# microsoft/NOTSOFAR1-Challenge

Hardware: AMD Instinct MI355X
Metric: CSS real-time-factor (sep. audio sec/wall sec) on 7-ch 16 kHz (higher is better)
Workload: dtype f32 (float32 operands on v_mfma_f32_32x32x2_f32 in every Linear layer, attention product and transform: the reference's own operand precision; MVDR covariance / solve f64)

## Files before the change

notsofar1-challenge_amd/csrc/encoder.hip:

```cpp
#include "kernels.hpp"
#include "split_f16.hpp"

namespace css {

typedef float f32x16 __attribute__((ext_vector_type(16)));
typedef _Float16 f16x8 __attribute__((ext_vector_type(8)));

template <int CTRL>
__device__ __forceinline__ float dpp_addf(float v) {
    return v + __int_as_float(__builtin_amdgcn_update_dpp(0, __float_as_int(v), CTRL, 0xf, 0xf, false));
}
__device__ __forceinline__ float wave_sum(float v) {
    v = dpp_addf<0xB1>(v);
    v = dpp_addf<0x4E>(v);
    v = dpp_addf<0x141>(v);
    v = dpp_addf<0x140>(v);
    const float r0 = __int_as_float(__builtin_amdgcn_readlane(__float_as_int(v), 0));
    const float r1 = __int_as_float(__builtin_amdgcn_readlane(__float_as_int(v), 16));
    const float r2 = __int_as_float(__builtin_amdgcn_readlane(__float_as_int(v), 32));
    const float r3 = __int_as_float(__builtin_amdgcn_readlane(__float_as_int(v), 48));
    return (r0 + r1) + (r2 + r3);
}

#ifndef CSS_LN_ROWS
#define CSS_LN_ROWS 4
#endif
constexpr int LN_ROWS = CSS_LN_ROWS;
template <int NV, int MODE>
__global__ __launch_bounds__(64 * LN_ROWS) void layernorm_kernel(const float* __restrict__ x, float* __restrict__ y,
                                                        float* __restrict__ ys, const float* __restrict__ w,
                                                        const float* __restrict__ b, const float* __restrict__ pw,
                                                        int rows) {
    constexpr int D = 256 * NV;
    const int row = blockIdx.x * LN_ROWS + (threadIdx.x >> 6);
    if (row >= rows) return;
    const int lane = threadIdx.x & 63;
    const float4* xr = reinterpret_cast<const float4*>(x + (int64_t)row * D);
    float4 v[NV];
    float s = 0.f;
#pragma unroll
    for (int i = 0; i < NV; ++i) {
        v[i] = xr[lane + 64 * i];
        s += (v[i].x + v[i].y) + (v[i].z + v[i].w);
    }
    const float mean = wave_sum(s) * (1.0f / D);
    float q = 0.f;
#pragma unroll
    for (int i = 0; i < NV; ++i) {
        v[i].x -= mean; v[i].y -= mean; v[i].z -= mean; v[i].w -= mean;
        q += (v[i].x * v[i].x + v[i].y * v[i].y) + (v[i].z * v[i].z + v[i].w * v[i].w);
    }
    const float rstd = 1.0f / sqrtf(wave_sum(q) * (1.0f / D) + 1e-5f);
    float p0 = 0.f, p1 = 0.f, p2 = 0.f, p3 = 0.f;
    if (MODE == 2) { p0 = pw[0]; p1 = pw[1]; p2 = pw[2]; p3 = pw[3]; }
    float4* yr = reinterpret_cast<float4*>(y + (int64_t)row * D);
    _Float16* ysr = reinterpret_cast<_Float16*>(ys + (int64_t)row * D);
#pragma unroll
    for (int i = 0; i < NV; ++i) {
        const float4 g = reinterpret_cast<const float4*>(w)[lane + 64 * i];
        const float4 be = reinterpret_cast<const float4*>(b)[lane + 64 * i];
        float o[4] = {v[i].x * rstd * g.x + be.x, v[i].y * rstd * g.y + be.y, v[i].z * rstd * g.z + be.z,
                      v[i].w * rstd * g.w + be.w};
#pragma unroll
        for (int e = 0; e < 4; ++e) {
            if (MODE == 1) o[e] = fmaxf(o[e], 0.f);
            if (MODE == 2) o[e] = (p0 * o[e] + p1) * (1.0f / (1.0f + expf(-(p2 * o[e] + p3))));
        }
        if (y) yr[lane + 64 * i] = make_float4(o[0], o[1], o[2], o[3]);
        if (ys) split_store4(ysr, 4 * (lane + 64 * i), o[0], o[1], o[2], o[3]);
    }
}

template <int NV>
__global__ __launch_bounds__(64 * LN_ROWS) void layernorm2_kernel(const float* __restrict__ x, float* __restrict__ y,
                                                         const float* __restrict__ w1, const float* __restrict__ b1,
                                                         float* __restrict__ z, float* __restrict__ zs,
                                                         const float* __restrict__ w2, const float* __restrict__ b2,
                                                         int rows) {
    constexpr int D = 256 * NV;
    const int row = blockIdx.x * LN_ROWS + (threadIdx.x >> 6);
    if (row >= rows) return;
    const int lane = threadIdx.x & 63;
    const float4* xr = reinterpret_cast<const float4*>(x + (int64_t)row * D);
    float4 v[NV];
#pragma unroll
    for (int i = 0; i < NV; ++i) v[i] = xr[lane + 64 * i];
#pragma unroll
    for (int pass = 0; pass < 2; ++pass) {
        float s = 0.f;
#pragma unroll
        for (int i = 0; i < NV; ++i) s += (v[i].x + v[i].y) + (v[i].z + v[i].w);
        const float mean = wave_sum(s) * (1.0f / D);
        float q = 0.f;
#pragma unroll
        for (int i = 0; i < NV; ++i) {
            v[i].x -= mean; v[i].y -= mean; v[i].z -= mean; v[i].w -= mean;
            q += (v[i].x * v[i].x + v[i].y * v[i].y) + (v[i].z * v[i].z + v[i].w * v[i].w);
        }
        const float rstd = 1.0f / sqrtf(wave_sum(q) * (1.0f / D) + 1e-5f);
        const float* w = pass ? w2 : w1;
        const float* b = pass ? b2 : b1;
        float* yo = pass ? z : y;
#pragma unroll
        for (int i = 0; i < NV; ++i) {
            const float4 g = reinterpret_cast<const float4*>(w)[lane + 64 * i];
            const float4 be = reinterpret_cast<const float4*>(b)[lane + 64 * i];
            v[i] = make_float4(v[i].x * rstd * g.x + be.x, v[i].y * rstd * g.y + be.y, v[i].z * rstd * g.z + be.z,
                               v[i].w * rstd * g.w + be.w);
            if (yo) reinterpret_cast<float4*>(yo + (int64_t)row * D)[lane + 64 * i] = v[i];
            if (pass && zs)
                split_store4(reinterpret_cast<_Float16*>(zs + (int64_t)row * D), 4 * (lane + 64 * i), v[i].x, v[i].y, v[i].z, v[i].w);
        }
    }
}

void launch_layernorm2(const float* x, float* y, const float* w1, const float* b1, float* z, float* z_split,
                       const float* w2, const float* b2, int rows, int D, hipStream_t s) {
    const dim3 grid((rows + LN_ROWS - 1) / LN_ROWS), block(64 * LN_ROWS);
    switch (D) {
        case 256: hipLaunchKernelGGL((layernorm2_kernel<1>), grid, block, 0, s, x, y, w1, b1, z, z_split, w2, b2, rows); break;
        case 512: hipLaunchKernelGGL((layernorm2_kernel<2>), grid, block, 0, s, x, y, w1, b1, z, z_split, w2, b2, rows); break;
        case 768: hipLaunchKernelGGL((layernorm2_kernel<3>), grid, block, 0, s, x, y, w1, b1, z, z_split, w2, b2, rows); break;
        case 1024: hipLaunchKernelGGL((layernorm2_kernel<4>), grid, block, 0, s, x, y, w1, b1, z, z_split, w2, b2, rows); break;
        default: break;
    }
}

template <int MODE>
static void launch_ln_mode(const float* x, float* y, float* ys, const float* w, const float* b, const float* pw,
                           int rows, int D, hipStream_t s) {
    const dim3 grid((rows + LN_ROWS - 1) / LN_ROWS), block(64 * LN_ROWS);
    switch (D) {
        case 256: hipLaunchKernelGGL((layernorm_kernel<1, MODE>), grid, block, 0, s, x, y, ys, w, b, pw, rows); break;
        case 512: hipLaunchKernelGGL((layernorm_kernel<2, MODE>), grid, block, 0, s, x, y, ys, w, b, pw, rows); break;
        case 768: hipLaunchKernelGGL((layernorm_kernel<3, MODE>), grid, block, 0, s, x, y, ys, w, b, pw, rows); break;
        case 1024: hipLaunchKernelGGL((layernorm_kernel<4, MODE>), grid, block, 0, s, x, y, ys, w, b, pw, rows); break;
        default: break;
    }
}

void launch_layernorm(const float* x, float* y, float* y_split, const float* w, const float* b, int rows, int D,
                      int relu, hipStream_t s) {
    if (relu) launch_ln_mode<1>(x, y, y_split, w, b, nullptr, rows, D, s);
    else launch_ln_mode<0>(x, y, y_split, w, b, nullptr, rows, D, s);
}

void launch_ln_glu(const float* x, float* z, const float* w, const float* b, const float* pw, int rows, int D,
                   hipStream_t s) {
    launch_ln_mode<2>(x, z, nullptr, w, b, pw, rows, D, s);
}

template <int TAPS, int RUN>
__global__ __launch_bounds__(256) void dwconv_kernel(const float* __restrict__ z, float* __restrict__ h,
                                                     const float* __restrict__ wt, const float* __restrict__ dwb,
                                                     const float* __restrict__ alpha, const float* __restrict__ beta,
                                                     const float* __restrict__ pw, int T, int D, int runs_per_seg) {
    constexpr int PAD = (TAPS - 1) / 2;
    const int ch = blockIdx.x * 256 + threadIdx.x;
    if (ch >= D) return;
    const int seg = blockIdx.y / runs_per_seg, run = blockIdx.y % runs_per_seg;
    const int t0 = run * RUN;
    const float* zs = z + (int64_t)seg * T * D + ch;
    float wk[TAPS];
#pragma clang loop unroll(full)
    for (int k = 0; k < TAPS; ++k) wk[k] = wt[k * D + ch];
    float acc[RUN];
#pragma clang loop unroll(full)
    for (int j = 0; j < RUN; ++j) acc[j] = 0.f;
#pragma clang loop unroll(full)
    for (int p = 0; p < RUN + TAPS - 1; ++p) {
        const int t = t0 + p - PAD;
        const float v = (t >= 0 && t < T) ? zs[(int64_t)t * D] : 0.f;
#pragma clang loop unroll(full)
        for (int j = (p - (TAPS - 1) > 0 ? p - (TAPS - 1) : 0); j <= (p < RUN - 1 ? p : RUN - 1); ++j)
            acc[j] = fmaf(wk[p - j], v, acc[j]);
    }
    const float bb = dwb[ch], al = alpha[ch], be = beta[ch], w2 = pw[4], c2 = pw[5];
    float* hs = h + (int64_t)seg * T * D + ch;
#pragma unroll
    for (int j = 0; j < RUN; ++j) {
        const int t = t0 + j;
        if (t < T) {
            const float y = fmaxf((acc[j] + bb) * al + be, 0.f);
            hs[(int64_t)t * D] += w2 * y + c2;
        }
    }
}

void launch_dwconv(const float* z, float* h, const float* dw_wt, const float* dw_b, const float* bn_alpha,
                   const float* bn_beta, const float* pw, int nseg, int T, int D, int taps, hipStream_t s) {
    constexpr int RUN = 31;
    const int runs = (T + RUN - 1) / RUN;
    const dim3 grid((D + 255) / 256, nseg * runs), block(256);
    if (taps == 33)
        hipLaunchKernelGGL((dwconv_kernel<33, RUN>), grid, block, 0, s, z, h, dw_wt, dw_b, bn_alpha, bn_beta, pw, T, D, runs);
    else if (taps == 31)
        hipLaunchKernelGGL((dwconv_kernel<31, RUN>), grid, block, 0, s, z, h, dw_wt, dw_b, bn_alpha, bn_beta, pw, T, D, runs);
    else if (taps == 17)
        hipLaunchKernelGGL((dwconv_kernel<17, RUN>), grid, block, 0, s, z, h, dw_wt, dw_b, bn_alpha, bn_beta, pw, T, D, runs);
}

template <int NV, int TAPS, int RUN, int HV>
__global__ __launch_bounds__(256 * NV * HV) void conv_module_kernel(const float* __restrict__ x_in, float* __restrict__ x_out,
                                                              const float* __restrict__ lnw, const float* __restrict__ lnb,
                                                              const float* __restrict__ pw, const float* __restrict__ wt,
                                                              const float* __restrict__ dwb, const float* __restrict__ alpha,
                                                              const float* __restrict__ beta,
                                                              const float* __restrict__ ln2w, const float* __restrict__ ln2b,
                                                              float* __restrict__ z, float* __restrict__ zs, int T, int runs_per_seg) {
    constexpr int D = 256 * NV, PAD = (TAPS - 1) / 2, ROWS = RUN + TAPS - 1, NW = 4 * NV * HV, JH = (RUN + HV - 1) / HV;
    extern __shared__ __attribute__((aligned(16))) float tile[];
    const int item = css_xcd_item((int)blockIdx.x, (int)gridDim.x);
    const int seg = item / runs_per_seg, run = item % runs_per_seg;
    const int t0 = run * RUN;
    const int wave = threadIdx.x >> 6, lane = threadIdx.x & 63;
    const float p0 = pw[0], p1 = pw[1], p2 = pw[2], p3 = pw[3];
    const int ch = threadIdx.x % D, j0 = (threadIdx.x / D) * JH;
    float wk[TAPS];
#pragma clang loop unroll(full)
    for (int k = 0; k < TAPS; ++k) wk[k] = wt[k * D + ch];
    const float bb = dwb[ch], al = alpha[ch], be_ = beta[ch], w2 = pw[4], c2 = pw[5];
    const float* xs = x_in + (int64_t)seg * T * D + ch;
    float xres[JH];
#pragma clang loop unroll(full)
    for (int j = 0; j < JH; ++j) xres[j] = xs[(int64_t)min(t0 + j0 + j, T - 1) * D];
    constexpr int RPW = (ROWS + NW - 1) / NW;
    float4 v[RPW][NV];
#pragma unroll
    for (int i = 0; i < RPW; ++i) {
        const int p = wave + i * NW, t = t0 + p - PAD;
        const bool ok = p < ROWS && t >= 0 && t < T;
        const float4* xr = reinterpret_cast<const float4*>(x_in + ((int64_t)seg * T + (ok ? t : 0)) * D);
#pragma unroll
        for (int j = 0; j < NV; ++j) v[i][j] = ok ? xr[lane + 64 * j] : make_float4(0.f, 0.f, 0.f, 0.f);
    }
#pragma unroll
    for (int i = 0; i < RPW; ++i) {
        const int p = wave + i * NW, t = t0 + p - PAD;
        if (p >= ROWS) break;
        float4* dst = reinterpret_cast<float4*>(tile + p * D);
        if (t < 0 || t >= T) {
#pragma unroll
            for (int j = 0; j < NV; ++j) dst[lane + 64 * j] = make_float4(0.f, 0.f, 0.f, 0.f);
            continue;
        }
        float s = 0.f;
#pragma unroll
        for (int j = 0; j < NV; ++j) s += (v[i][j].x + v[i][j].y) + (v[i][j].z + v[i][j].w);
        const float mean = wave_sum(s) * (1.0f / D);
        float q = 0.f;
#pragma unroll
        for (int j = 0; j < NV; ++j) {
            v[i][j].x -= mean; v[i][j].y -= mean; v[i][j].z -= mean; v[i][j].w -= mean;
            q += (v[i][j].x * v[i][j].x + v[i][j].y * v[i][j].y) + (v[i][j].z * v[i][j].z + v[i][j].w * v[i][j].w);
        }
        const float rstd = 1.0f / sqrtf(wave_sum(q) * (1.0f / D) + 1e-5f);
#pragma unroll
        for (int j = 0; j < NV; ++j) {
            const float4 g = reinterpret_cast<const float4*>(lnw)[lane + 64 * j];
            const float4 be = reinterpret_cast<const float4*>(lnb)[lane + 64 * j];
            float o[4] = {v[i][j].x * rstd * g.x + be.x, v[i][j].y * rstd * g.y + be.y, v[i][j].z * rstd * g.z + be.z,
                          v[i][j].w * rstd * g.w + be.w};
#pragma unroll
            for (int e = 0; e < 4; ++e) {
                const float z = p2 * o[e] + p3;
                o[e] = (p0 * o[e] + p1) * __builtin_amdgcn_rcpf(1.0f + __builtin_amdgcn_exp2f(z * -1.44269504088896341f));
            }
            dst[lane + 64 * j] = make_float4(o[0], o[1], o[2], o[3]);
        }
    }
    __syncthreads();
    float acc[JH];
#pragma clang loop unroll(full)
    for (int j = 0; j < JH; ++j) acc[j] = 0.f;
#pragma clang loop unroll(full)
    for (int pp = 0; pp < JH + TAPS - 1; ++pp) {
        const float zv = tile[min(j0 + pp, ROWS - 1) * D + ch];
#pragma clang loop unroll(full)
        for (int j = (pp - (TAPS - 1) > 0 ? pp - (TAPS - 1) : 0); j <= (pp < JH - 1 ? pp : JH - 1); ++j)
            acc[j] = fmaf(wk[pp - j], zv, acc[j]);
    }
    __syncthreads();
#pragma unroll
    for (int j = 0; j < JH; ++j) {
        const float y = fmaxf((acc[j] + bb) * al + be_, 0.f);
        if (j0 + j < RUN) tile[(j0 + j) * D + ch] = xres[j] + (w2 * y + c2);
    }
    __syncthreads();
    for (int j = wave; j < RUN && t0 + j < T; j += NW) {
        const int64_t row = (int64_t)seg * T + t0 + j;
        float4 r[NV];
        float s = 0.f;
#pragma unroll
        for (int i = 0; i < NV; ++i) {
            r[i] = reinterpret_cast<const float4*>(tile + j * D)[lane + 64 * i];
            reinterpret_cast<float4*>(x_out + row * D)[lane + 64 * i] = r[i];
            s += (r[i].x + r[i].y) + (r[i].z + r[i].w);
        }
        if (!z && !zs) continue;
        const float mean = wave_sum(s) * (1.0f / D);
        float q = 0.f;
#pragma unroll
        for (int i = 0; i < NV; ++i) {
            r[i].x -= mean; r[i].y -= mean; r[i].z -= mean; r[i].w -= mean;
            q += (r[i].x * r[i].x + r[i].y * r[i].y) + (r[i].z * r[i].z + r[i].w * r[i].w);
        }
        const float rstd = 1.0f / sqrtf(wave_sum(q) * (1.0f / D) + 1e-5f);
#pragma unroll
        for (int i = 0; i < NV; ++i) {
            const float4 g = reinterpret_cast<const float4*>(ln2w)[lane + 64 * i];
            const float4 be = reinterpret_cast<const float4*>(ln2b)[lane + 64 * i];
            const float4 o = make_float4(r[i].x * rstd * g.x + be.x, r[i].y * rstd * g.y + be.y, r[i].z * rstd * g.z + be.z,
                                         r[i].w * rstd * g.w + be.w);
            if (z) reinterpret_cast<float4*>(z + row * D)[lane + 64 * i] = o;
            if (zs) split_store4(reinterpret_cast<_Float16*>(zs + row * D), 4 * (lane + 64 * i), o.x, o.y, o.z, o.w);
        }
    }
}

bool launch_conv_module(const float* x_in, float* x_out, const float* ln_w, const float* ln_b, const float* pw,
                        const float* dw_wt, const float* dw_b, const float* bn_alpha, const float* bn_beta,
                        const float* ln2_w, const float* ln2_b, float* z, float* z_split, int nseg, int T,
                        int D, int taps, hipStream_t s) {
#ifndef CSS_CONV_RUN
#define CSS_CONV_RUN 31
#endif
    constexpr int RUN = CSS_CONV_RUN;
    if (taps != 33 || (D != 256 && D != 512)) return false;
    const int runs = (T + RUN - 1) / RUN;
    const size_t lds = (size_t)(RUN + 32) * D * sizeof(float);
    const void* fn = D == 512 ? reinterpret_cast<const void*>(&conv_module_kernel<2, 33, RUN, 2>)
                              : reinterpret_cast<const void*>(&conv_module_kernel<1, 33, RUN, 2>);
    if (hipFuncSetAttribute(fn, hipFuncAttributeMaxDynamicSharedMemorySize, 160 * 1024) != hipSuccess) {
        (void)hipGetLastError();
        return false;
    }
    if (D == 512)
        hipLaunchKernelGGL((conv_module_kernel<2, 33, RUN, 2>), dim3(nseg * runs), dim3(1024), lds, s, x_in, x_out, ln_w, ln_b, pw, dw_wt,
                           dw_b, bn_alpha, bn_beta, ln2_w, ln2_b, z, z_split, T, runs);
    else
        hipLaunchKernelGGL((conv_module_kernel<1, 33, RUN, 2>), dim3(nseg * runs), dim3(512), lds, s, x_in, x_out, ln_w, ln_b, pw, dw_wt,
                           dw_b, bn_alpha, bn_beta, ln2_w, ln2_b, z, z_split, T, runs);
    return true;
}

template <int NJT, bool QKS, bool FRAG, int W>
__global__ __launch_bounds__(64 * W, (NJT <= 7 ? 2 : 1)) void relpos_attn_kernel(const float* __restrict__ qkv, const float* __restrict__ qkf,
                                                         const float* __restrict__ pe,
                                                         float* __restrict__ ctx, int T, int D, int maxlen,
                                                         int split_out, int heads, int n_items) {
    constexpr int DK = 64;
    constexpr int LDR = 98;
    const int wv = W > 1 ? __builtin_amdgcn_readfirstlane((int)(threadIdx.x >> 6)) : 0;
    __shared__ __attribute__((aligned(16))) float lds_all[W][32 * LDR];
    float (&lds)[32 * LDR] = lds_all[wv];
    const int item = css_xcd_item((int)blockIdx.x, (int)gridDim.x) * W + wv;
    if (item >= n_items) return;
    const int qt = item % NJT, head = (item / NJT) % heads, seg = item / (NJT * heads);
    const int lane = threadIdx.x & 63, c = lane & 31, h = lane >> 5;
    const int ld = 3 * D;
    const float* qb = qkv + (int64_t)seg * T * ld + head * DK;
    const float* kb = qb + D;
    const float* vb = qb + 2 * D;
    const int i0 = qt * 32;
    const int iq = min(i0 + c, T - 1);

    float4 q[8];
#define CSS_ATT_LOAD8(dst, rowptr)                                                                      \
    _Pragma("unroll") for (int ch = 0; ch < 8; ++ch)                                                    \
        dst[ch] = *reinterpret_cast<const float4*>((rowptr) + (QKS ? ((ch >> 2) * 32 + ((ch >> 1) & 1) * 8 + (ch & 1) * 16) : 8 * ch) + 4 * h);
    const float4* qkt = reinterpret_cast<const float4*>(qkf) +
                        ((int64_t)(seg * heads + head) * NJT) * (2 * 8 * 64) + lane;
    if constexpr (FRAG) {
#pragma unroll
        for (int ch = 0; ch < 8; ++ch) q[ch] = qkt[(qt * 2 + 0) * 512 + ch * 64];
    } else {
        CSS_ATT_LOAD8(q, qb + (int64_t)iq * ld)
    }

    const int rel0 = i0 - (T - 1);
    auto pe_tile = [&](int rt) { return pe + ((int64_t)(qt + rt) * 8 * 64 + lane) * 4; };
    auto k_row = [&](int jt) { return kb + (int64_t)min(jt * 32 + c, T - 1) * ld; };
    (void)rel0; (void)maxlen;

    constexpr int RT0 = NJT;
    constexpr int NPRO = NJT >= 2 ? 3 : 2;
    constexpr int NI = NJT >= 2 ? NJT - 2 : 0;
    constexpr int NS = NPRO + NJT + NI;
    auto step_rt = [](int s_) {
        if (s_ < NPRO) return RT0 - s_;
        const int u_ = s_ - NPRO;
        return (u_ < 2 * NI && (u_ & 1)) ? RT0 - 3 - (u_ >> 1) : -1;
    };
    auto step_jt = [](int s_) {
        const int u_ = s_ - NPRO;
        return u_ < 2 * NI ? (u_ >> 1) : NI + (u_ - 2 * NI);
    };
#define CSS_ATT_LOAD_STEP(dst, s_)                                                                         \
    {                                                                                                      \
        if (step_rt(s_) >= 0) {                                                                            \
            const float4* pt_ = reinterpret_cast<const float4*>(pe_tile(step_rt(s_)));                     \
            _Pragma("unroll") for (int ch = 0; ch < 8; ++ch) dst[ch] = pt_[ch * 64];                       \
        } else if constexpr (FRAG) {                                                                       \
            _Pragma("unroll") for (int ch = 0; ch < 8; ++ch) dst[ch] = qkt[(step_jt(s_) * 2 + 1) * 512 + ch * 64]; \
        } else {                                                                                           \
            CSS_ATT_LOAD8(dst, k_row(step_jt(s_)))                                                         \
        }                                                                                                  \
    }
    constexpr int NTB = 2;
    float4 tb[NTB][8];
    f32x16 S[NJT];
    int step = 0;
#define CSS_ATT_LOAD_CH(dst, s_, ch)                                                                       \
    {                                                                                                      \
        if (step_rt(s_) >= 0) dst[ch] = reinterpret_cast<const float4*>(pe_tile(step_rt(s_)))[(ch) * 64];  \
        else if constexpr (FRAG) dst[ch] = qkt[(step_jt(s_) * 2 + 1) * 512 + (ch) * 64];                   \
        else dst[ch] = *reinterpret_cast<const float4*>(k_row(step_jt(s_)) + (QKS ? (((ch) >> 2) * 32 + (((ch) >> 1) & 1) * 8 + ((ch) & 1) * 16) : 8 * (ch)) + 4 * h); \
    }
#define CSS_ATT_STEP(acc)                                                                                  \
    {                                                                                                      \
        __builtin_amdgcn_sched_barrier(0);                                                                 \
        _Pragma("unroll") for (int r = 0; r < 16; ++r) acc[r] = 0.f;                                       \
        f32x16 cor_ = {0};                                                                                 \
        _Pragma("unroll") for (int ch = 0; ch < 8; ++ch) {                                                 \
            if (step + NTB - 1 < NS) { CSS_ATT_LOAD_CH(tb[(step + NTB - 1) % NTB], min(step + NTB - 1, NS - 1), ch) } \
            const float4 s4_ = tb[step % NTB][ch];                                                         \
            if constexpr (QKS) {    \
                if (ch & 1) {                                                                              \
                    const f16x8 sh_ = __builtin_bit_cast(f16x8, tb[step % NTB][ch - 1]), sl_ = __builtin_bit_cast(f16x8, s4_); \
                    const f16x8 qh_ = __builtin_bit_cast(f16x8, q[ch - 1]), ql_ = __builtin_bit_cast(f16x8, q[ch]);         \
                    acc = __builtin_amdgcn_mfma_f32_32x32x16_f16(sh_, qh_, acc, 0, 0, 0);                  \
                    cor_ = __builtin_amdgcn_mfma_f32_32x32x16_f16(sh_, ql_, cor_, 0, 0, 0);                \
                    cor_ = __builtin_amdgcn_mfma_f32_32x32x16_f16(sl_, qh_, cor_, 0, 0, 0);                \
                    __builtin_amdgcn_sched_barrier(0);                                                     \
                }                                                                                          \
            } else {                                                                                       \
                acc = __builtin_amdgcn_mfma_f32_32x32x2f32(s4_.x, q[ch].x, acc, 0, 0, 0);                  \
                acc = __builtin_amdgcn_mfma_f32_32x32x2f32(s4_.y, q[ch].y, acc, 0, 0, 0);                  \
                acc = __builtin_amdgcn_mfma_f32_32x32x2f32(s4_.z, q[ch].z, acc, 0, 0, 0);                  \
                acc = __builtin_amdgcn_mfma_f32_32x32x2f32(s4_.w, q[ch].w, acc, 0, 0, 0);                  \
                __builtin_amdgcn_sched_barrier(0);                                                         \
            }                                                                                              \
        }                                                                                                  \
        if constexpr (QKS) acc += cor_ * SPLIT_LO_INV;                                                     \
        __builtin_amdgcn_sched_barrier(0);                                                                 \
        ++step;                                                                                            \
    }
#define CSS_ATT_RING_WRITE(acc, rt)                                                          \
    {                                                                                        \
        const int slot_ = (((rt) % 3) + 3) % 3;                                              \
        _Pragma("unroll") for (int r = 0; r < 16; ++r)                                       \
            lds[c * LDR + slot_ * 32 + (r & 3) + 8 * (r >> 2) + 4 * h] = acc[r];             \
    }
    CSS_ATT_LOAD_STEP(tb[0], 0)
    if constexpr (NTB > 2) { CSS_ATT_LOAD_STEP(tb[1], 1) }
#pragma unroll
    for (int u = 0; u < NPRO; ++u) {
        const int rt = RT0 - u;
        f32x16 acc;
        CSS_ATT_STEP(acc)
        CSS_ATT_RING_WRITE(acc, rt)
    }
    float mx = -INFINITY;
    const int base_c = c + (T - 1) - 4 * h;
    const int m0 = base_c >= 0 ? base_c % 96 : 0;
    const float* ringc = lds + c * LDR;
#pragma unroll
    for (int jt = 0; jt < NJT; ++jt) {
        const int rt_new = RT0 - 3 - jt;
        CSS_ATT_STEP(S[jt])
#pragma unroll
        for (int r = 0; r < 16; ++r) {
            const int K = jt * 32 + (r & 3) + 8 * (r >> 2);
            float bpos, sc;
            if (jt < NJT - 1) {
                const unsigned t = (unsigned)(m0 - K % 96);
                bpos = ringc[min(t, t + 96u)];
                sc = S[jt][r] + bpos;
            } else {
                const int rr = max(base_c - K, 0);
                bpos = ringc[((rr >> 5) % 3) * 32 + (rr & 31)];
                sc = S[jt][r] + bpos;
                sc = K + 4 * h < T ? sc : -INFINITY;
            }
            S[jt][r] = sc;
            mx = fmaxf(mx, sc);
        }
        if (rt_new >= 0) {
            f32x16 acc;
            CSS_ATT_STEP(acc)
            CSS_ATT_RING_WRITE(acc, rt_new)
        }
    }
    mx = fmaxf(mx, __shfl_xor(mx, 32));
    const float c1 = 0.125f * 1.44269504088896341f, mc = mx * c1;
    float sum = 0.f;
#pragma unroll
    for (int jt = 0; jt < NJT; ++jt) {
#pragma unroll
        for (int r = 0; r < 16; ++r) {
            const float p = __builtin_amdgcn_exp2f(fmaf(S[jt][r], c1, -mc));
            S[jt][r] = p;
            sum += p;
        }
    }
    sum += __shfl_xor(sum, 32);
    const float inv = 1.0f / sum;
    __builtin_amdgcn_fence(__ATOMIC_RELEASE, "wavefront");
    __builtin_amdgcn_wave_barrier();

    constexpr int OLD = 65;
    if constexpr (QKS) {
        typedef __fp16 h4 __attribute__((__vector_size__(4 * sizeof(__fp16))));
        constexpr int VIMG = 32 * 32;
        constexpr int VLO = VIMG + 32;
        constexpr int VBUF = VLO + VIMG;
        static_assert(2 * VBUF * sizeof(_Float16) <= sizeof(lds), "V tile buffers must fit in the ring");
        _Float16* vlds = reinterpret_cast<_Float16*>(lds);
        float4 vr[4];
        const int vkey = lane >> 3, vpc = lane & 7;
#define CSS_ATT_VLOAD(g_)                                                                                          \
    _Pragma("unroll") for (int m = 0; m < 4; ++m) {                                                               \
        const int ju_ = ((g_) >> 1) * 32 + 8 * m + vkey;                                                          \
        const int row_ = ((g_) >> 1) < NJT - 1 ? ju_ : min(ju_, T - 1);                                           \
        vr[m] = *reinterpret_cast<const float4*>(vb + (int64_t)row_ * ld + ((g_) & 1) * 32 + 4 * vpc);            \
    }
#define CSS_ATT_VSTORE(g_)                                                                                         \
    _Pragma("unroll") for (int m = 0; m < 4; ++m)                                                                 \
        *reinterpret_cast<float4*>(vlds + ((g_) & 1) * VBUF + (vpc >> 2) * VLO + (8 * m + vkey) * 32 + (vpc & 3) * 8) = vr[m];
        const int tq = c >> 4, ti = c & 15;
        const int troff = (4 * h + (ti >> 2)) * 32 + 16 * tq + 4 * (ti & 3);
#define CSS_ATT_TR(g_, img_, kk_, eh_)                                                                             \
    __builtin_amdgcn_ds_read_tr16_b64_v4f16(reinterpret_cast<__attribute__((address_space(3))) h4*>(              \
        (__attribute__((address_space(3))) _Float16*)vlds + ((g_) & 1) * VBUF + (img_) * VLO + (16 * (kk_) + 8 * (eh_)) * 32 + troff))
        CSS_ATT_VLOAD(0)
        CSS_ATT_VSTORE(0)
        CSS_ATT_VLOAD(1)
        f32x16 o0 = {0}, o1 = {0}, cor0 = {0}, cor1 = {0};
#pragma unroll
        for (int jt = 0; jt < NJT; ++jt) {
            f16x8 ph[2], pl[2];
#pragma unroll
            for (int kk = 0; kk < 2; ++kk)
#pragma unroll
                for (int e = 0; e < 8; ++e) {
                    _Float16 a, b;
                    split_f16(S[jt][8 * kk + e], a, b);
                    ph[kk][e] = a;
                    pl[kk][e] = b;
                }
#pragma unroll
            for (int dt = 0; dt < 2; ++dt) {
                const int g = 2 * jt + dt;
                if (g + 1 < 2 * NJT) { CSS_ATT_VSTORE(g + 1) }
                if (g + 2 < 2 * NJT) { CSS_ATT_VLOAD(g + 2) }
#pragma unroll
                for (int kk = 0; kk < 2; ++kk) {
                    const h4 a0 = CSS_ATT_TR(g, 0, kk, 0), a1 = CSS_ATT_TR(g, 0, kk, 1);
                    const h4 b0 = CSS_ATT_TR(g, 1, kk, 0), b1 = CSS_ATT_TR(g, 1, kk, 1);
                    f16x8 vh, vl;
#pragma unroll
                    for (int e = 0; e < 4; ++e) {
                        vh[e] = (_Float16)a0[e]; vh[4 + e] = (_Float16)a1[e];
                        vl[e] = (_Float16)b0[e]; vl[4 + e] = (_Float16)b1[e];
                    }
                    if (dt == 0) {
                        o0 = __builtin_amdgcn_mfma_f32_32x32x16_f16(vh, ph[kk], o0, 0, 0, 0);
                        cor0 = __builtin_amdgcn_mfma_f32_32x32x16_f16(vh, pl[kk], cor0, 0, 0, 0);
                        cor0 = __builtin_amdgcn_mfma_f32_32x32x16_f16(vl, ph[kk], cor0, 0, 0, 0);
                    } else {
                        o1 = __builtin_amdgcn_mfma_f32_32x32x16_f16(vh, ph[kk], o1, 0, 0, 0);
                        cor1 = __builtin_amdgcn_mfma_f32_32x32x16_f16(vh, pl[kk], cor1, 0, 0, 0);
                        cor1 = __builtin_amdgcn_mfma_f32_32x32x16_f16(vl, ph[kk], cor1, 0, 0, 0);
                    }
                }
            }
        }
        o0 += cor0 * SPLIT_LO_INV;
        o1 += cor1 * SPLIT_LO_INV;
#pragma unroll
        for (int r = 0; r < 16; ++r) {
            const int d = (r & 3) + 8 * (r >> 2) + 4 * h;
            lds[c * OLD + d] = o0[r] * inv;
            lds[c * OLD + 32 + d] = o1[r] * inv;
        }
#undef CSS_ATT_VLOAD
#undef CSS_ATT_VSTORE
#undef CSS_ATT_TR
    } else {
    typedef float f32x2 __attribute__((ext_vector_type(2)));
    f32x2 vb2[2][16];
    const __amdgpu_buffer_rsrc_t rsv = __builtin_amdgcn_make_buffer_rsrc(const_cast<float*>(vb), 0, (int)(((int64_t)(T - 1) * ld + DK) * 4), 0x00020000);
    const int vvo = (4 * h * ld + 2 * c) * 4, ldb = ld * 4;
#define CSS_ATT_LOADV(jt_, r_) __builtin_bit_cast(f32x2, __builtin_amdgcn_raw_buffer_load_b64(rsv, vvo, ((jt_) * 32 + ((r_) & 3) + 8 * ((r_) >> 2)) * ldb, 0))
#pragma unroll
    for (int r = 0; r < 16; ++r) vb2[0][r] = CSS_ATT_LOADV(0, r);
    f32x16 oe = {0}, oo = {0};
#pragma unroll
    for (int jt = 0; jt < NJT; ++jt) {
        __builtin_amdgcn_sched_barrier(0);
#pragma unroll
        for (int r = 0; r < 16; ++r) {
            if (jt + 1 < NJT) vb2[(jt + 1) & 1][r] = CSS_ATT_LOADV(jt + 1, r);
            oe = __builtin_amdgcn_mfma_f32_32x32x2f32(vb2[jt & 1][r].x, S[jt][r], oe, 0, 0, 0);
            oo = __builtin_amdgcn_mfma_f32_32x32x2f32(vb2[jt & 1][r].y, S[jt][r], oo, 0, 0, 0);
            __builtin_amdgcn_sched_barrier(0);
        }
    }
#pragma unroll
    for (int r = 0; r < 16; ++r) {
        const int d = 2 * ((r & 3) + 8 * (r >> 2) + 4 * h);
        lds[c * OLD + d] = oe[r] * inv;
        lds[c * OLD + d + 1] = oo[r] * inv;
    }
#undef CSS_ATT_LOADV
    }
    __builtin_amdgcn_fence(__ATOMIC_RELEASE, "wavefront");
    __builtin_amdgcn_wave_barrier();
    {
        const int d4 = (lane & 15) * 4;
        float* ob = ctx + ((int64_t)seg * T + i0) * D;
#pragma unroll
        for (int k = 0; k < 8; ++k) {
            const int il = (lane >> 4) + 4 * k;
            if (i0 + il >= T) continue;
            const float* src = lds + il * OLD + d4;
            const float v0 = src[0], v1 = src[1], v2 = src[2], v3 = src[3];
            if (split_out)
                split_store4(reinterpret_cast<_Float16*>(ob + (int64_t)il * D), head * DK + d4, v0, v1, v2, v3);
            else
                *reinterpret_cast<float4*>(ob + (int64_t)il * D + head * DK + d4) = make_float4(v0, v1, v2, v3);
        }
    }
}

__global__ __launch_bounds__(256) void relpos_attn_long_kernel(const float* __restrict__ qkv, const float* __restrict__ pe,
                                                               float* __restrict__ ctx, int T, int D, int maxlen, int split_out,
                                                               int heads, int nq) {
    constexpr int DK = 64;
    extern __shared__ __attribute__((aligned(16))) float att_lds[];
    const int qtiles = (T + nq - 1) / nq;
    const int item = blockIdx.x;
    const int qt = item % qtiles, head = (item / qtiles) % heads, seg = item / (qtiles * heads);
    const int i0 = qt * nq, nv = min(nq, T - i0);
    float* qs = att_lds;
    float* ss = qs + nq * DK;
    const int tid = threadIdx.x;
    const int64_t ld = 3 * (int64_t)D;
    const float* base = qkv + (int64_t)seg * T * ld + head * DK;
    for (int e = tid; e < nv * DK; e += 256) qs[e] = base[(int64_t)(i0 + e / DK) * ld + (e % DK)];
    __syncthreads();
    const int sub = tid & 3, kq = tid >> 2;
    auto quad_sum = [](float v) {
        v += __int_as_float(__builtin_amdgcn_update_dpp(0, __float_as_int(v), 0xB1, 0xf, 0xf, false));
        v += __int_as_float(__builtin_amdgcn_update_dpp(0, __float_as_int(v), 0x4E, 0xf, 0xf, false));
        return v;
    };
    auto load_row = [&](const float* rowp, float (&row)[16]) {
#pragma unroll
        for (int m = 0; m < 4; ++m) {
            const float4 v = *reinterpret_cast<const float4*>(rowp + 16 * m + 4 * sub);
            row[4 * m] = v.x; row[4 * m + 1] = v.y; row[4 * m + 2] = v.z; row[4 * m + 3] = v.w;
        }
    };
    auto dots4 = [&](int i, const float (&row)[16], float (&acc)[4]) {
#pragma unroll
        for (int k = 0; k < 4; ++k) acc[k] = 0.f;
#pragma unroll
        for (int m = 0; m < 4; ++m)
#pragma unroll
            for (int k = 0; k < 4; ++k) {
                const float4 q = *reinterpret_cast<const float4*>(qs + min(i + k, nv - 1) * DK + 16 * m + 4 * sub);
                acc[k] = fmaf(q.x, row[4 * m], acc[k]); acc[k] = fmaf(q.y, row[4 * m + 1], acc[k]);
                acc[k] = fmaf(q.z, row[4 * m + 2], acc[k]); acc[k] = fmaf(q.w, row[4 * m + 3], acc[k]);
            }
#pragma unroll
        for (int k = 0; k < 4; ++k) acc[k] = quad_sum(acc[k]);
    };
    for (int j0 = 0; j0 < T; j0 += 64) {
        const int j = j0 + kq;
        float row[16];
        load_row(base + (int64_t)min(j, T - 1) * ld + D, row);
        for (int i = 0; i < nv; i += 4) {
            float acc[4];
            dots4(i, row, acc);
            const float mine = sub == 0 ? acc[0] : sub == 1 ? acc[1] : sub == 2 ? acc[2] : acc[3];
            if (j < T && i + sub < nv) ss[(size_t)(i + sub) * T + j] = mine;
        }
    }
    __syncthreads();
    const int nu = nv + T - 1;
    for (int u0 = 0; u0 < nu; u0 += 64) {
        const int u = u0 + kq;
        const int rel = max(-maxlen, min(i0 - (T - 1) + u, maxlen - 1)) + maxlen;
        float row[16];
        load_row(pe + (int64_t)rel * DK, row);
        for (int i = 0; i < nv; i += 4) {
            float acc[4];
            dots4(i, row, acc);
            const float mine = sub == 0 ? acc[0] : sub == 1 ? acc[1] : sub == 2 ? acc[2] : acc[3];
            const int j = i + sub + T - 1 - u;
            if (u < nu && i + sub < nv && j >= 0 && j < T) ss[(size_t)(i + sub) * T + j] = (ss[(size_t)(i + sub) * T + j] + mine) * 0.125f;
        }
    }
    __syncthreads();
    const int wave = tid >> 6, lane = tid & 63;
    for (int i = wave; i < nv; i += 4) {
        float* row = ss + (size_t)i * T;
        float mx = -INFINITY;
        for (int j = lane; j < T; j += 64) mx = fmaxf(mx, row[j]);
#pragma unroll
        for (int o = 32; o > 0; o >>= 1) mx = fmaxf(mx, __shfl_xor(mx, o));
        float sum = 0.f;
        for (int j = lane; j < T; j += 64) { const float e = expf(row[j] - mx); row[j] = e; sum += e; }
        sum = wave_sum(sum);
        const float inv = 1.0f / sum;
        for (int j = lane; j < T; j += 64) row[j] *= inv;
    }
    __syncthreads();
    {
        const int d = tid & 63, ig = tid >> 6;
        constexpr int MAXQ = 4;
        float acc[MAXQ] = {0.f, 0.f, 0.f, 0.f};
        const float* vb = base + 2 * D + d;
#pragma unroll 8
        for (int j = 0; j < T; ++j) {
            const float v = vb[(int64_t)j * ld];
#pragma unroll
            for (int k = 0; k < MAXQ; ++k) {
                const int i = ig + 4 * k;
                if (i < nv) acc[k] = fmaf(ss[(size_t)i * T + j], v, acc[k]);
            }
        }
        float* ob = ctx + ((int64_t)seg * T + i0) * D;
#pragma unroll
        for (int k = 0; k < MAXQ; ++k) {
            const int i = ig + 4 * k;
            if (i >= nv) continue;
            if (split_out) split_store(reinterpret_cast<_Float16*>(ob + (int64_t)i * D), head * DK + d, acc[k]);
            else ob[(int64_t)i * D + head * DK + d] = acc[k];
        }
    }
}

bool launch_relpos_attention_long(const float* qkv, const float* pe, float* ctx, int nseg, int T, int D, int H, int maxlen,
                                  int split_out, hipStream_t s) {
    if (D != H * 64) return false;
    int nq = 16;
    auto bytes = [&](int n) { return ((size_t)n * 64 + (size_t)n * T) * sizeof(float); };
    while (nq > 1 && bytes(nq) > 52 * 1024) nq >>= 1;
    if (bytes(nq) > 150 * 1024) return false;
    if (bytes(nq) > 65536 && hipFuncSetAttribute(reinterpret_cast<const void*>(relpos_attn_long_kernel),
                                                 hipFuncAttributeMaxDynamicSharedMemorySize, (int)bytes(nq)) != hipSuccess)
        return false;
    const unsigned qtiles = (unsigned)((T + nq - 1) / nq);
    hipLaunchKernelGGL(relpos_attn_long_kernel, dim3(qtiles * (unsigned)H * (unsigned)nseg), dim3(256), bytes(nq), s, qkv, pe, ctx, T, D,
                       maxlen, split_out, H, nq);
    return true;
}

__global__ __launch_bounds__(256) void pe_fragments_kernel(const float* __restrict__ pe, float* __restrict__ frag, int T,
                                                           int maxlen, int ntiles, int split) {
    const int i = blockIdx.x * 256 + threadIdx.x;
    if (i >= ntiles * 8 * 64) return;
    const int lane = i & 63, ch = (i >> 6) & 7, m = i >> 9;
    const int c = lane & 31, h = lane >> 5;
    int prow = 32 * m - (T - 1) + c;
    prow = max(-maxlen, min(prow, maxlen - 1)) + maxlen;
    const int off = (split ? ((ch >> 2) * 32 + ((ch >> 1) & 1) * 8 + (ch & 1) * 16) : 8 * ch) + 4 * h;
    reinterpret_cast<float4*>(frag)[i] = *reinterpret_cast<const float4*>(pe + (int64_t)prow * 64 + off);
}

void launch_pe_fragments(const float* pe, float* frag, int T, int maxlen, int split, hipStream_t s) {
    const int ntiles = pe_fragment_tiles(T);
    hipLaunchKernelGGL(pe_fragments_kernel, dim3((ntiles * 8 * 64 + 255) / 256), dim3(256), 0, s, pe, frag, T, maxlen, ntiles, split);
}

#ifndef CSS_ATT_WAVES
#define CSS_ATT_WAVES 4
#endif
void launch_relpos_attention(const float* qkv, const float* qk_frag, const float* pe_frag, float* ctx, int nseg, int T, int D,
                             int H, int maxlen, int qk_split, int split_out, hipStream_t s) {
    const int qtiles = (T + 31) / 32;
    const int n_items = qtiles * H * nseg;
#define CSS_ATT_LAUNCH(n, w)                                                                                                 \
    {                                                                                                                        \
        const dim3 grid((unsigned)((n_items + (w) - 1) / (w))), block(64 * (w));                                              \
        if (qk_split && qk_frag) hipLaunchKernelGGL((relpos_attn_kernel<n, true, true, w>), grid, block, 0, s, qkv, qk_frag, pe_frag, ctx, T, D, maxlen, split_out, H, n_items);  \
        else if (qk_split) hipLaunchKernelGGL((relpos_attn_kernel<n, true, false, w>), grid, block, 0, s, qkv, qk_frag, pe_frag, ctx, T, D, maxlen, split_out, H, n_items);  \
        else hipLaunchKernelGGL((relpos_attn_kernel<n, false, false, w>), grid, block, 0, s, qkv, qk_frag, pe_frag, ctx, T, D, maxlen, split_out, H, n_items);          \
    }
#define CSS_ATT_CASE(n) case n: CSS_ATT_LAUNCH(n, (n <= 7 ? CSS_ATT_WAVES : 1)) break;
    switch (qtiles) {
        CSS_ATT_CASE(1) CSS_ATT_CASE(2) CSS_ATT_CASE(3) CSS_ATT_CASE(4)
        CSS_ATT_CASE(5) CSS_ATT_CASE(6) CSS_ATT_CASE(7) CSS_ATT_CASE(8)
        CSS_ATT_CASE(9) CSS_ATT_CASE(10) CSS_ATT_CASE(11) CSS_ATT_CASE(12)
        CSS_ATT_CASE(13) CSS_ATT_CASE(14) CSS_ATT_CASE(15) CSS_ATT_CASE(16)
        default: break;
    }
#undef CSS_ATT_CASE
#undef CSS_ATT_LAUNCH
}

}
```

Baseline: 7327.

## Interleave relpos bias consume and softmax exp with MFMA steps in attention

Reworks the relative-position attention kernel so the bias-add, masking and max reduction for each key tile run inside the MFMA loop of the next tile. The exp/sum softmax pass is likewise spread across the PV MFMA loop. The LDS ring is widened with a duplicated slot so reads need no modulo wrap, and the K-row clamp is skipped for non-final tiles. The goal is to hide the VALU and LDS work behind the matrix-core instructions. In exchange it uses more LDS per wave and keeps more registers live, which could lower occupancy.

```diff
diff --git a/notsofar1-challenge_amd/csrc/encoder.hip b/notsofar1-challenge_amd/csrc/encoder.hip
--- a/notsofar1-challenge_amd/csrc/encoder.hip
+++ b/notsofar1-challenge_amd/csrc/encoder.hip
@@ -350,7 +350,7 @@
                                                          float* __restrict__ ctx, int T, int D, int maxlen,
                                                          int split_out, int heads, int n_items) {
     constexpr int DK = 64;
-    constexpr int LDR = 98;
+    constexpr int LDR = 130;
     const int wv = W > 1 ? __builtin_amdgcn_readfirstlane((int)(threadIdx.x >> 6)) : 0;
     __shared__ __attribute__((aligned(16))) float lds_all[W][32 * LDR];
     float (&lds)[32 * LDR] = lds_all[wv];
@@ -380,7 +380,7 @@
 
     const int rel0 = i0 - (T - 1);
     auto pe_tile = [&](int rt) { return pe + ((int64_t)(qt + rt) * 8 * 64 + lane) * 4; };
-    auto k_row = [&](int jt) { return kb + (int64_t)min(jt * 32 + c, T - 1) * ld; };
+    auto k_row = [&](int jt) { return kb + (int64_t)(jt < NJT - 1 ? jt * 32 + c : min(jt * 32 + c, T - 1)) * ld; };
     (void)rel0; (void)maxlen;
 
     constexpr int RT0 = NJT;
@@ -417,7 +417,9 @@
         else if constexpr (FRAG) dst[ch] = qkt[(step_jt(s_) * 2 + 1) * 512 + (ch) * 64];                   \
         else dst[ch] = *reinterpret_cast<const float4*>(k_row(step_jt(s_)) + (QKS ? (((ch) >> 2) * 32 + (((ch) >> 1) & 1) * 8 + ((ch) & 1) * 16) : 8 * (ch)) + 4 * h); \
     }
-#define CSS_ATT_STEP(acc)                                                                                  \
+#define CSS_ATT_NO_FILL(g_)
+#define CSS_ATT_STEP(acc) CSS_ATT_STEP_FILL(acc, CSS_ATT_NO_FILL)
+#define CSS_ATT_STEP_FILL(acc, FILL)                                                                       \
     {                                                                                                      \
         __builtin_amdgcn_sched_barrier(0);                                                                 \
         _Pragma("unroll") for (int r = 0; r < 16; ++r) acc[r] = 0.f;                                       \
@@ -432,6 +434,7 @@
                     acc = __builtin_amdgcn_mfma_f32_32x32x16_f16(sh_, qh_, acc, 0, 0, 0);                  \
                     cor_ = __builtin_amdgcn_mfma_f32_32x32x16_f16(sh_, ql_, cor_, 0, 0, 0);                \
                     cor_ = __builtin_amdgcn_mfma_f32_32x32x16_f16(sl_, qh_, cor_, 0, 0, 0);                \
+                    FILL(ch >> 1)                                                                          \
                     __builtin_amdgcn_sched_barrier(0);                                                     \
                 }                                                                                          \
             } else {                                                                                       \
@@ -439,6 +442,7 @@
                 acc = __builtin_amdgcn_mfma_f32_32x32x2f32(s4_.y, q[ch].y, acc, 0, 0, 0);                  \
                 acc = __builtin_amdgcn_mfma_f32_32x32x2f32(s4_.z, q[ch].z, acc, 0, 0, 0);                  \
                 acc = __builtin_amdgcn_mfma_f32_32x32x2f32(s4_.w, q[ch].w, acc, 0, 0, 0);                  \
+                FILL(ch)                                                                                   \
                 __builtin_amdgcn_sched_barrier(0);                                                         \
             }                                                                                              \
         }                                                                                                  \
@@ -449,8 +453,10 @@
 #define CSS_ATT_RING_WRITE(acc, rt)                                                          \
     {                                                                                        \
         const int slot_ = (((rt) % 3) + 3) % 3;                                              \
-        _Pragma("unroll") for (int r = 0; r < 16; ++r)                                       \
+        _Pragma("unroll") for (int r = 0; r < 16; ++r) {                                     \
             lds[c * LDR + slot_ * 32 + (r & 3) + 8 * (r >> 2) + 4 * h] = acc[r];             \
+            if (slot_ == 0) lds[c * LDR + 96 + (r & 3) + 8 * (r >> 2) + 4 * h] = acc[r];     \
+        }                                                                                    \
     }
     CSS_ATT_LOAD_STEP(tb[0], 0)
     if constexpr (NTB > 2) { CSS_ATT_LOAD_STEP(tb[1], 1) }
@@ -461,51 +467,68 @@
         CSS_ATT_STEP(acc)
         CSS_ATT_RING_WRITE(acc, rt)
     }
+    if constexpr (NJT == 1) {
+#pragma unroll
+        for (int r = 0; r < 16; ++r) lds[c * LDR + 64 + (r & 3) + 8 * (r >> 2) + 4 * h] = 0.f;
+    }
     float mx = -INFINITY;
-    const int base_c = c + (T - 1) - 4 * h;
-    const int m0 = base_c >= 0 ? base_c % 96 : 0;
-    const float* ringc = lds + c * LDR;
+    auto wrap96 = [](int t) { return (int)min((unsigned)t, (unsigned)t + 96u); };
+    const int m0 = wrap96(wrap96(c - 4 * h + (T - 1) % 96) - 96);
+    const int s0 = wrap96(m0 - 27), s1 = wrap96(s0 - 32), s2 = wrap96(s1 - 32);
+    const int klim = T - 32 * (NJT - 1) - 4 * h;
+    const float* const ringc = lds + c * LDR;
+    const float* const ring3[3] = {ringc + s0, ringc + s1, ringc + s2};
+    float bp[16];
+#define CSS_ATT_RING_READ(jt_)                                                                             \
+    _Pragma("unroll") for (int r = 0; r < 16; ++r) bp[r] = ring3[(jt_) % 3][27 - ((r & 3) + 8 * (r >> 2))];
+#define CSS_ATT_CONSUME(jt_, r_)                                                                           \
+    {                                                                                                      \
+        float sc_ = S[jt_][r_] + bp[r_];                                                                   \
+        if ((jt_) == NJT - 1) sc_ = ((r_) & 3) + 8 * ((r_) >> 2) < klim ? sc_ : -INFINITY;                 \
+        S[jt_][r_] = sc_;                                                                                  \
+        mx = fmaxf(mx, sc_);                                                                               \
+    }
+    constexpr int NPG = QKS ? 4 : 2;
+#define CSS_ATT_CONSUME_PREV(g_) _Pragma("unroll") for (int e_ = 0; e_ < NPG; ++e_) CSS_ATT_CONSUME(jt - 1, NPG * (g_) + e_)
+#define CSS_ATT_CONSUME_THIS(g_) _Pragma("unroll") for (int e_ = 0; e_ < NPG; ++e_) CSS_ATT_CONSUME(jt, NPG * (g_) + e_)
 #pragma unroll
     for (int jt = 0; jt < NJT; ++jt) {
         const int rt_new = RT0 - 3 - jt;
-        CSS_ATT_STEP(S[jt])
-#pragma unroll
-        for (int r = 0; r < 16; ++r) {
-            const int K = jt * 32 + (r & 3) + 8 * (r >> 2);
-            float bpos, sc;
-            if (jt < NJT - 1) {
-                const unsigned t = (unsigned)(m0 - K % 96);
-                bpos = ringc[min(t, t + 96u)];
-                sc = S[jt][r] + bpos;
-            } else {
-                const int rr = max(base_c - K, 0);
-                bpos = ringc[((rr >> 5) % 3) * 32 + (rr & 31)];
-                sc = S[jt][r] + bpos;
-                sc = K + 4 * h < T ? sc : -INFINITY;
-            }
-            S[jt][r] = sc;
-            mx = fmaxf(mx, sc);
-        }
+        if (jt >= 1 && rt_new + 1 < 0) {
+            CSS_ATT_STEP_FILL(S[jt], CSS_ATT_CONSUME_PREV)
+        } else {
+            CSS_ATT_STEP(S[jt])
+        }
+        CSS_ATT_RING_READ(jt)
         if (rt_new >= 0) {
             f32x16 acc;
-            CSS_ATT_STEP(acc)
+            CSS_ATT_STEP_FILL(acc, CSS_ATT_CONSUME_THIS)
             CSS_ATT_RING_WRITE(acc, rt_new)
-        }
-    }
+        } else if (jt == NJT - 1) {
+#pragma unroll
+            for (int r = 0; r < 16; ++r) CSS_ATT_CONSUME(jt, r)
+        }
+    }
+#undef CSS_ATT_RING_READ
+#undef CSS_ATT_CONSUME_PREV
+#undef CSS_ATT_CONSUME_THIS
+#undef CSS_ATT_CONSUME
     mx = fmaxf(mx, __shfl_xor(mx, 32));
     const float c1 = 0.125f * 1.44269504088896341f, mc = mx * c1;
-    float sum = 0.f;
-#pragma unroll
-    for (int jt = 0; jt < NJT; ++jt) {
-#pragma unroll
-        for (int r = 0; r < 16; ++r) {
-            const float p = __builtin_amdgcn_exp2f(fmaf(S[jt][r], c1, -mc));
-            S[jt][r] = p;
-            sum += p;
-        }
-    }
-    sum += __shfl_xor(sum, 32);
-    const float inv = 1.0f / sum;
+    float sum = 0.f, inv = 0.f;
+#define CSS_ATT_PROB(jt_, r_)                                                          \
+    {                                                                                  \
+        const float p_ = __builtin_amdgcn_exp2f(fmaf(S[jt_][r_], c1, -mc));            \
+        S[jt_][r_] = p_;                                                               \
+        sum += p_;                                                                     \
+    }
+#define CSS_ATT_CLOSE_SUM()                                                            \
+    {                                                                                  \
+        sum += __shfl_xor(sum, 32);                                                    \
+        inv = 1.0f / sum;                                                              \
+    }
+#pragma unroll
+    for (int r = 0; r < 16; ++r) CSS_ATT_PROB(0, r)
     __builtin_amdgcn_fence(__ATOMIC_RELEASE, "wavefront");
     __builtin_amdgcn_wave_barrier();
 
@@ -573,6 +596,12 @@
                         cor1 = __builtin_amdgcn_mfma_f32_32x32x16_f16(vh, pl[kk], cor1, 0, 0, 0);
                         cor1 = __builtin_amdgcn_mfma_f32_32x32x16_f16(vl, ph[kk], cor1, 0, 0, 0);
                     }
+                    if (jt + 1 < NJT) {
+#pragma unroll
+                        for (int e = 0; e < 4; ++e) CSS_ATT_PROB(jt + 1, 4 * (2 * dt + kk) + e)
+                    } else if (dt == 0 && kk == 0) {
+                        CSS_ATT_CLOSE_SUM()
+                    }
                 }
             }
         }
@@ -604,6 +633,8 @@
             if (jt + 1 < NJT) vb2[(jt + 1) & 1][r] = CSS_ATT_LOADV(jt + 1, r);
             oe = __builtin_amdgcn_mfma_f32_32x32x2f32(vb2[jt & 1][r].x, S[jt][r], oe, 0, 0, 0);
             oo = __builtin_amdgcn_mfma_f32_32x32x2f32(vb2[jt & 1][r].y, S[jt][r], oo, 0, 0, 0);
+            if (jt + 1 < NJT) CSS_ATT_PROB(jt + 1, r)
+            else if (r == 0) CSS_ATT_CLOSE_SUM()
             __builtin_amdgcn_sched_barrier(0);
         }
     }
@@ -615,6 +646,8 @@
     }
 #undef CSS_ATT_LOADV
     }
+#undef CSS_ATT_PROB
+#undef CSS_ATT_CLOSE_SUM
     __builtin_amdgcn_fence(__ATOMIC_RELEASE, "wavefront");
     __builtin_amdgcn_wave_barrier();
     {
```

Result: no change. 7385, median of 6 (+0.8%).
